# theislab/dca

Measured on NVIDIA H100. Metric: cells/sec (ZINB AE epoch, device-timed), higher is better.
Workload: dtype bf16-gemm/f32-acc/f32-loss

## Files before the change

dca_b200/_lib.py:

```python
from __future__ import annotations

import ctypes as C
import os

_HERE = os.path.dirname(os.path.abspath(__file__))
LIB_PATH = os.path.join(_HERE, "libdca_b200.so")

DCA_MAX_HIDDEN = 8
DCA_NAME_LEN = 48

ACTIVATION_IDS = {"relu": 0, "linear": 1, "elu": 2, "selu": 3, "tanh": 4, "sigmoid": 5, "hard_sigmoid": 6,
                  "softplus": 7, "softsign": 8, "exponential": 9, "LeakyReLU": 10, "PReLU": 11}
OPTIMIZERS = {"RMSprop": (0, 1e-3), "SGD": (1, 1e-2), "Adagrad": (2, 1e-2), "Adadelta": (3, 1.0), "Adam": (4, 1e-3),
              "Adamax": (5, 2e-3), "Nadam": (6, 2e-3)}
OPTIMIZERS.update({k.lower(): v for k, v in list(OPTIMIZERS.items())})
AE_TYPE_IDS = {"zinb-conddisp": 0, "zinb": 1, "nb-conddisp": 2, "nb": 3,
               "poisson": 4, "normal": 5, "nb-shared": 6, "zinb-shared": 7, "zinb-elempi": 8, "nb-fork": 9, "zinb-fork": 10}
F32, BF16 = 0, 1
GEMM_AUTO, GEMM_GENERIC, GEMM_TCGEN05 = 0, 1, 2
REGION_PARAMS, REGION_GRADS, REGION_RMS, REGION_BN_STATE, REGION_EPOCH_ACC = 0, 1, 2, 3, 4


class DcaError(RuntimeError):
    pass
# ... 61 lines not shown
    "dca_train_step_host": (C.c_int, [_vp, _vp, _vp, _vp, _i32, _f, _f, C.POINTER(_f), _vp]),
    "dca_set_input_transform": (C.c_int, [_vp, _vp, _vp, _i32, _i32, _vp]),
    "dca_set_loss_ring": (C.c_int, [_vp, _vp, _i32]),
    "dca_stream_begin": (C.c_int, [_vp, _vp, _i64, _vp, _i64, _i32, _vp]),
    "dca_stream_begin_packed": (C.c_int, [_vp, _vp, _i32, _i64, _vp, _vp, _vp, _i64, _i32, _vp]),
    "dca_stream_begin_sparse": (C.c_int, [_vp, _vp, _vp, _vp, _vp, _vp, _vp, _i64, _i32, _vp]),
    "dca_stream_step": (C.c_int, [_vp, _i64, _i64, _vp]),
    "dca_stream_end": (C.c_int, [_vp, _vp]),
    "dca_expand_packed_counts": (C.c_int, [_vp, _i32, _vp, _vp, _vp, _i32, _i32, _vp, _vp, _i32, _i32, _vp, _vp, _i32, _vp,
                                           _vp]),
    "dca_expand_sparse_counts": (C.c_int, [_vp, _vp, _vp, _i32, _vp, _vp, _vp, _i32, _i32, _vp, _vp, _i32, _i32, _vp, _vp,
                                           _i32, _vp, _vp]),
    "dca_zinb_loss_fwd_bwd": (C.c_int, [_vp, _i64, _vp, _vp, _vp, _vp, _vp, _i64, _i32, _i32, _i32, _f, _f,
                                        _vp, _vp, _vp, _i32, _vp, _vp, _vp, _sz, _vp]),
    "dca_zinb_loss_workspace_bytes": (C.c_int, [_i32, _i32, C.POINTER(_sz)]),
    "dca_zinb_loss_fwd": (C.c_int, [_vp, _i64, _vp, _vp, _vp, _vp, _vp, _i64, _i32, _i32, _i32, _f,
                                    _vp, _vp, _sz, _vp]),
    "dca_zinb_elem_host": (C.c_int, [_i32, _f, _f, _f, _f, _f, _f, C.POINTER(_f * 4)]),
    "dca_dropout_mask_host": (C.c_int, [C.c_uint64, C.c_uint64, _i32, _i64, _f, _vp]),
    "dca_activation_host": (C.c_int, [_i32, _f, _f, C.POINTER(_f * 2)]),
    "dca_activation_bwd_host": (C.c_int, [_i32, _f, _f, _f, _i32, _f, C.POINTER(_f * 2)]),
    "dca_dense_heads_fwd": (C.c_int, [_vp, _i64, _i32, _i32, _i32, _vp, _vp, _vp, _vp, _vp, _vp, _vp,
                                      _vp, _vp, _vp, _i64, _vp]),
    "dca_tc_heads_fwd": (C.c_int, [_vp, _i32, _vp, _vp, _i32, _i32, C.POINTER(_i32 * 3), _vp, _vp, _vp, _vp, _i64, _vp]),
    "dca_tc_heads_loss": (C.c_int, [_vp, _i32, _vp, _vp, _i32, _vp, _i64, _vp, _vp, _f, _f, _vp, _vp, _vp, _i64, _vp,
                                    _vp, _sz, _vp]),
    "dca_tc_gene_gemm": (C.c_int, [_i32, _vp, _vp, _vp, _i64, _i32, _i32, _i32, _vp, _vp, _vp, _vp, _vp, _vp, _i64, _i32,
                                   _vp, _vp, _vp, _vp]),
    "dca_tc_gene_gemm_sms": (C.c_int, [_i32, _vp, _vp, _vp, _i64, _i32, _i32, _i32, _vp, _vp, _vp, _vp, _vp, _vp, _i64,
                                       _i32, _vp, _vp, _vp, _vp, _i32]),
    "dca_tc_gene_gemm_rows": (C.c_int, [_i32, _vp, _vp, _vp, _i64, _vp, _i32, _i32, _i32, _vp, _vp, _vp, _vp, _vp, _vp,
                                        _i64, _i32, _vp, _vp, _vp, _vp, _i32]),
    "dca_head_bwd_schedule": (C.c_int, [_i32, _i32, _i32, _i32, _i32, _vp, _i64, C.POINTER(_i64), _vp]),
    "dca_enc_bwd_schedule": (C.c_int, [_i32, _i32, _vp, _i64, _vp]),
    "dca_tc_probe": (C.c_int, [_vp, _i32, _i32, _vp, _i32, _i32, _i32, _i32, _i32, _i32, _i32, _i32, _i32, _i32, _i32,
                               _vp, _vp]),
    "dca_profile_enable": (C.c_int, [_vp, _i32]),
    "dca_profile_read": (C.c_int, [_vp, C.POINTER(C.c_double * 6), C.POINTER(C.c_int64 * 6), _i32]),
    "dca_engine_info": (C.c_int, [_vp, C.POINTER(_i32 * 8)]),
    "dca_write_text_matrix": (C.c_int, [C.c_char_p, _vp, _i32, _i64, _i64, _i64, _vp, _vp, _i32, _i32]),
    "dca_write_text_device": (C.c_int, [C.c_char_p, _i32, _vp, _i64, _i64, _i64, _i32, _vp, _i64, _vp, _vp, _i64, _i32, _vp,
                                        _vp]),
    "dca_format_fixed6_host": (C.c_int, [_vp, _i64, _vp, _vp]),
    "dca_read_text_counts": (C.c_int, [C.c_char_p, _i32, _i32, _i64, _i32, _vp, _vp, _i64, _vp, _vp, _i64, _vp]),
    "dca_read_mtx_counts": (C.c_int, [C.c_char_p, _i32, _i64, _i32, _vp, _vp, _vp, _vp, _vp]),
    "dca_read_text_counts_gz": (C.c_int, [C.c_char_p, _i32, _i32, _i64, _i32, _vp, _vp, _i64, _vp, _vp, _i64, _vp]),
    "dca_read_mtx_counts_gz": (C.c_int, [C.c_char_p, _i32, _i64, _i32, _vp, _vp, _vp, _vp, _vp]),
    "dca_gunzip": (C.c_int, [C.c_char_p, _i32, _vp, _vp, _i64, _vp]),
    "dca_inflate_span_host": (C.c_int, [_vp, _i64, _i32, _i64, _i64, _vp, _i64, _vp]),
    "dca_inflate_find_host": (C.c_int, [_vp, _i64, _i64, _i64, _vp]),
    "dca_count_escapes": (C.c_int, [_vp, _i32, _i64, _i64, _i64, _vp, _i32]),
    "dca_pack_counts": (C.c_int, [_vp, _i32, _i64, _i64, _i64, _i32, _vp, _vp, _vp, _i32]),
    "dca_sparse_counts": (C.c_int, [_vp, _i32, _i64, _i64, _i64, _vp, _vp, _i32]),
    "dca_pack_sparse": (C.c_int, [_vp, _i32, _i64, _i64, _i64, _vp, _vp, _vp, _vp, _vp, _i32]),
    "dca_preprocess_workspace_bytes": (C.c_int, [_i64, _i32, C.POINTER(_sz)]),
    "dca_counts_csr_to_dense": (C.c_int, [_vp, _vp, _vp, _i64, _i32, _vp, _i64, _vp]),
    "dca_count_totals": (C.c_int, [_vp, _i64, _i64, _i32, _vp, _vp, _vp, _vp, _sz, _vp]),
    "dca_gather_counts": (C.c_int, [_vp, _i64, _vp, _i64, _vp, _i32, _vp, _i64, _vp]),
    "dca_log_moments": (C.c_int, [_vp, _i64, _i64, _i32, _vp, C.c_double, _i32, _vp, _vp, _vp, _sz, _vp]),
    "dca_normalize_write": (C.c_int, [_vp, _i64, _i64, _i32, _vp, C.c_double, _i32, _vp, _vp, _vp, _i32, _i64, _vp]),
    "dca_stats_workspace_bytes": (C.c_int, [_i64, _i32, _i64, C.POINTER(_sz)]),
    "dca_stats_begin": (C.c_int, [_i64, _i32, _vp, _sz, _vp]),
    "dca_count_totals_rows": (C.c_int, [_vp, _i64, _i64, _i64, _i64, _i32, _vp, _vp, _sz, _vp]),
    "dca_count_totals_finish": (C.c_int, [_i64, _i32, _vp, _vp, _vp, _sz, _vp]),
    "dca_log_moments_rows": (C.c_int, [_i32, _vp, _i64, _i64, _i64, _i64, _i32, _vp, C.c_double, _i32, _vp, _vp, _sz,
                                       _vp]),
# ... 58 lines not shown
```

dca_b200/csrc/gene_gemm_tc.cu:

```cuda
#include "engine.h"
#include "tc_common.cuh"

namespace dca {
namespace tc {
int g_gg_profile = 0;
int g_head_bwd_banded = 1;
int g_head_bwd_stagger = 1300;
namespace gg {

constexpr int kThreads = 256;
constexpr uint32_t kZBytes = 128 * 128 * 2;
constexpr uint32_t kWBytes = 64 * 128 * 2;
constexpr uint32_t kHBytes = 128 * 64 * 2;
constexpr uint32_t kOutBytes = 128 * 64 * 4;
constexpr uint32_t kOnesBytes = 16 * 128;
constexpr int kMaxGb = 4;
constexpr int kMaxSlots = 16;

static_assert(kWBytes == kHBytes, "the two item kinds of the banded launch share one stage shape");
template <bool DO_A, bool DO_B, bool BANDED>
constexpr int stages() { return DO_A && DO_B && !BANDED ? 2 : 3; }
template <bool DO_A, bool DO_B, bool BANDED>
constexpr uint32_t stage_bytes() { return BANDED ? kZBytes + kWBytes : kZBytes + (DO_B ? kWBytes : 0) + (DO_A ? kHBytes : 0); }
template <bool DO_A, bool DO_B, bool COLSUM, bool BANDED>
constexpr uint32_t smem_bytes() {
  return stages<DO_A, DO_B, BANDED>() * stage_bytes<DO_A, DO_B, BANDED>() + (DO_A ? kOutBytes : 0) + (COLSUM ? kOnesBytes : 0) + 1024;
}

struct BandItem { int kind, head, gr, gb0, ng, cb0, ncb; };

__host__ __device__ inline BandItem band_item(int k, int n_gb, int n_cb, int gpr, int ranges) {
  const int per_head = n_gb + ranges * n_cb, full_band = gpr + n_cb;
  BandItem it;
  it.head = k / per_head; k -= it.head * per_head;
  it.gr = min(k / full_band, ranges - 1); k -= it.gr * full_band;
  const int gb0 = it.gr * gpr, ng = min(n_gb, gb0 + gpr) - gb0, m = min(ng, n_cb);
  int idx;
  if (k < 2 * m) { it.kind = k & 1; idx = k >> 1; }
  else { it.kind = ng > n_cb ? 0 : 1; idx = k - m; }
  if (it.kind == 0) { it.gb0 = gb0 + idx; it.ng = 1; it.cb0 = 0; it.ncb = n_cb; }
  else { it.gb0 = gb0; it.ng = ng; it.cb0 = idx; it.ncb = 1; }
  return it;
}

struct Params {
  int B, G, n_heads;
  int n_cb, n_gb;
  int gb_per_item, cb_per_item;
  int gene_ranges, cell_splits;
  int total_items;
  int stagger;
  float* db[3];
  float* part; int64_t part_stride;
  const int32_t* rows; const __nv_bfloat16* zsrc; int64_t ldz;
};

__device__ __forceinline__ void cp_async_16(uint32_t smem_dst, const void* src, uint32_t src_bytes) {
  asm volatile("cp.async.cg.shared.global [%0], [%1], 16, %2;" ::"r"(smem_dst), "l"(src), "r"(src_bytes) : "memory");
}
__device__ __forceinline__ void cp_async_commit() { asm volatile("cp.async.commit_group;" ::: "memory"); }
template <int N>
__device__ __forceinline__ void cp_async_wait() { asm volatile("cp.async.wait_group %0;" ::"n"(N) : "memory"); }

template <bool DO_A, bool DO_B, bool COLSUM, bool WK, int MAXG, bool BANDED>
__global__ void __launch_bounds__(kThreads, 1)
gene_gemm_kernel(const __grid_constant__ CUtensorMap map_z0, const __grid_constant__ CUtensorMap map_z1,
                 const __grid_constant__ CUtensorMap map_z2, const __grid_constant__ CUtensorMap map_h,
                 const __grid_constant__ CUtensorMap map_w0, const __grid_constant__ CUtensorMap map_w1,
                 const __grid_constant__ CUtensorMap map_w2, const __grid_constant__ CUtensorMap map_dw0, const __grid_constant__ CUtensorMap map_dw1,
                 const __grid_constant__ CUtensorMap map_dw2, const int dw_transposed, const Params p) {
  static_assert(!BANDED || (DO_A && DO_B && MAXG == 1), "banded items hold one gene block of (a) accumulators");
  constexpr int kStages = stages<DO_A, DO_B, BANDED>();
  constexpr uint32_t kStage = stage_bytes<DO_A, DO_B, BANDED>();
  constexpr uint32_t kHOff = kZBytes + (DO_B && !BANDED ? kWBytes : 0);
  extern __shared__ __align__(1024) uint8_t smem_raw[];
  uint8_t* smem = smem_raw + ((1024u - (smem_u32(smem_raw) & 1023u)) & 1023u);
  uint8_t* s_st = smem;
  float* s_o = reinterpret_cast<float*>(s_st + kStages * kStage);
  uint8_t* s_ones = reinterpret_cast<uint8_t*>(s_o) + (DO_A ? kOutBytes : 0);
  __shared__ uint64_t full[kStages];

  if (threadIdx.x == 0) {
    for (int i = 0; i < kStages; ++i) mbar_init(&full[i], 1);
    fence_barrier_init();
// ... 220 lines not shown
    const float4 v = __ldcs(reinterpret_cast<const float4*>(part + sl * stride + i));
    acc.x += v.x; acc.y += v.y; acc.z += v.z; acc.w += v.w;
  }
  *reinterpret_cast<float4*>(out + i) = acc;
}

void plan_a(Params& p, int n_heads, int sm_count) {
  int best_gpi = 1; long long best_cost = -1;
  for (int gpi = 1; gpi <= kMaxGb; ++gpi) {
    const long long items = (long long)cdiv(p.n_gb, gpi) * n_heads, rounds = (items + sm_count - 1) / sm_count;
    const long long cost = rounds * ((long long)gpi * p.n_cb + 2ll * gpi);
    if (best_cost < 0 || cost < best_cost) { best_cost = cost; best_gpi = gpi; }
  }
  p.gb_per_item = best_gpi; p.gene_ranges = cdiv(p.n_gb, best_gpi);
  p.cb_per_item = p.n_cb; p.cell_splits = 1;
  p.total_items = p.gene_ranges * n_heads;
}
void plan_b(Params& p, int n_heads, int sm_count) {
  p.cb_per_item = 1; p.cell_splits = p.n_cb;
  int gsplits = cdiv(4 * sm_count, p.n_cb * n_heads); if (gsplits < 1) gsplits = 1;
  if (gsplits > kMaxSlots / n_heads) gsplits = kMaxSlots / n_heads;
  if (gsplits > p.n_gb) gsplits = p.n_gb;
  while (gsplits > 1 && cdiv(p.n_gb, gsplits) < 4) --gsplits;
  p.gb_per_item = cdiv(p.n_gb, gsplits); p.gene_ranges = cdiv(p.n_gb, p.gb_per_item);
  p.total_items = p.gene_ranges * p.cell_splits * n_heads;
}
void plan_banded(Params& p, int n_heads, int sm_count, int* grid) {
  plan_b(p, n_heads, sm_count);
  p.total_items = n_heads * (p.n_gb + p.gene_ranges * p.n_cb);
  const int band = p.gb_per_item + p.n_cb;
  *grid = min(p.total_items, sm_count >= band ? sm_count / band * band : sm_count);
}

constexpr int kEbMaxW = 3;
constexpr int kEbThreads = 128 * kEbMaxW;
constexpr uint32_t kEbSub = 128 * 128;
constexpr uint32_t kEbStage = kEbMaxW * kEbSub + kHBytes;
constexpr int kEbStages = 3;
constexpr uint32_t kEbSmem = kEbStages * kEbStage + 1024;
static_assert(kEbMaxW * 64 * 64 * 4 <= kEbStage, "the flush staging tiles fit in the first stage");

struct EncBwdParams {
  int B, G, n_cb, n_blk;
  const int32_t* rows; const __nv_bfloat16* zsrc; int64_t ldz;
};

__host__ __device__ inline int eb_first(int c, int n_blk, int ctas) { return c * (n_blk / ctas) + min(c, n_blk % ctas); }
inline int eb_ctas(int n_blk, int sm_count) { return max(1, min(sm_count, n_blk)); }

__global__ void __launch_bounds__(kEbThreads, 1)
gene_gemm_enc_bwd_kernel(const __grid_constant__ CUtensorMap map_z, const __grid_constant__ CUtensorMap map_h,
                         const __grid_constant__ CUtensorMap map_dw, const int dw_transposed, const EncBwdParams p) {
  extern __shared__ __align__(1024) uint8_t smem_raw[];
  uint8_t* s_st = smem_raw + ((1024u - (smem_u32(smem_raw) & 1023u)) & 1023u);
  __shared__ uint64_t full[kEbStages];
  if (threadIdx.x == 0) {
    for (int i = 0; i < kEbStages; ++i) mbar_init(&full[i], 1);
    fence_barrier_init();
  }
  __syncthreads();

  const int wg = threadIdx.x >> 7, w = (threadIdx.x >> 5) & 3, l = threadIdx.x & 31;
  const int frow = 16 * w + (l >> 2), fcol = 2 * (l & 3);
  const bool gather = p.rows != nullptr;
  const int g_r0 = (threadIdx.x & 127) >> 3, g_c = threadIdx.x & 7;
  const uint32_t g_dst = wg * kEbSub + g_r0 * 128 + ((g_c ^ (g_r0 & 7)) << 4);
  int src_row[8];

  const int last = eb_first(blockIdx.x + 1, p.n_blk, gridDim.x);
  uint32_t T0 = 0;
  for (int blk0 = eb_first(blockIdx.x, p.n_blk, gridDim.x); blk0 < last; blk0 += kEbMaxW) {
    const int nw = min(kEbMaxW, last - blk0);
    const bool mine = wg < nw;
    if (threadIdx.x == 0) bulk_wait_read<0>();
    __syncthreads();

    auto issue = [&](int t) {
      const int st = (T0 + t) % kEbStages;
      uint8_t* dst = s_st + st * kEbStage;
      mbar_expect_tx(&full[st], kHBytes + (gather ? 0u : nw * kEbSub));
// ... 111 lines not shown
    for (int i = 0; i < 3; ++i) {
      float* d = dW[i < n_heads ? i : 0];
      if (dW_transposed) DCA_TRY(make_tensor_map_2d(&mdw[i], d, 4, 0, 64, (uint64_t)G, (uint64_t)dW_ld, 64, 128, 0));
      else {
        if (dW_ld != 64) { set_error("gene_gemm_tc: non-transposed dW needs ld == 64"); return DCA_ERR_BAD_ARG; }
        DCA_TRY(make_tensor_map_2d(&mdw[i], d, 4, 0, (uint64_t)G, 64, 64, 128, 64, 0));
      }
    }
  }
  if (do_b) {
    for (int i = 0; i < 3; ++i) {
      const __nv_bfloat16* w = W[i < n_heads ? i : 0];
      if (mode == 3) DCA_TRY(make_tensor_map_2d(&mw[i], w, 2, 1, 64, (uint64_t)G, (uint64_t)G, 64, 64, 1));
      else DCA_TRY(make_tensor_map_2d(&mw[i], w, 2, 1, (uint64_t)G, 64, 64, 128, 64, 1));
    }
  }
  Params base{};
  base.B = B; base.G = G; base.n_heads = n_heads;
  base.n_cb = cdiv(B, 128); base.n_gb = cdiv(G, 128);
  for (int i = 0; i < 3; ++i) base.db[i] = db ? db[i] : nullptr;
  base.part = reinterpret_cast<float*>(ws); base.part_stride = (int64_t)base.n_cb * 128 * 64;
  base.rows = rows; base.zsrc = Z[0]; base.ldz = ldz;

#define DCA_GG_LAUNCH(P, GRID, A, Bb, Cc, WKk, MG, BND)                                                                \
  do {                                                                                                                 \
    static bool attr = false;                                                                                          \
    constexpr uint32_t sm = smem_bytes<A, Bb, Cc, BND>();                                                              \
    if (!attr) { DCA_CUDA_OK(cudaFuncSetAttribute(gene_gemm_kernel<A, Bb, Cc, WKk, MG, BND>, cudaFuncAttributeMaxDynamicSharedMemorySize, (int)sm)); attr = true; } \
    gene_gemm_kernel<A, Bb, Cc, WKk, MG, BND><<<GRID, kThreads, sm, s>>>(mz[0], mz[1], mz[2], mh, mw[0], mw[1], mw[2],  \
                                                                          mdw[0], mdw[1], mdw[2], dW_transposed, P);  \
    DCA_LAUNCH_CHECK();                                                                                                \
  } while (0)

  if (mode == 3 && g_head_bwd_banded) {
    Params p = base;
    int grid = 0;
    plan_banded(p, n_heads, sm_count, &grid);
    p.stagger = g_head_bwd_stagger;
    DCA_GG_LAUNCH(p, grid, true, true, true, true, 1, true);
    const int64_t n = (int64_t)B * 64;
    gene_gemm_reduce_kernel<<<(unsigned)cdiv(n / 4, 256), 256, 0, s>>>(p.part, p.gene_ranges * n_heads, p.part_stride, out_b, n);
    DCA_LAUNCH_CHECK();
    return DCA_OK;
  }
  if (mode == 2) {
    EncBwdParams p{B, G, base.n_cb, cdiv(G, 64), rows, Z[0], ldz};
    CUtensorMap mdw64;
    if (dW_transposed) DCA_TRY(make_tensor_map_2d(&mdw64, dW[0], 4, 0, 64, (uint64_t)G, (uint64_t)dW_ld, 64, 64, 0));
    else DCA_TRY(make_tensor_map_2d(&mdw64, dW[0], 4, 0, (uint64_t)G, 64, 64, 64, 64, 0));
    static bool attr = false;
    if (!attr) { DCA_CUDA_OK(cudaFuncSetAttribute(gene_gemm_enc_bwd_kernel, cudaFuncAttributeMaxDynamicSharedMemorySize, (int)kEbSmem)); attr = true; }
    gene_gemm_enc_bwd_kernel<<<eb_ctas(p.n_blk, sm_count), kEbThreads, kEbSmem, s>>>(mz[0], mh, mdw64, dW_transposed, p);
    DCA_LAUNCH_CHECK();
    return DCA_OK;
  }
  if (do_a) {
    Params p = base;
    plan_a(p, n_heads, sm_count);
    DCA_GG_LAUNCH(p, min(p.total_items, sm_count), true, false, true, false, kMaxGb, false);
  }
  if (do_b) {
    Params p = base;
    plan_b(p, n_heads, sm_count);
    const int grid = min(p.total_items, sm_count);
    if (mode == 3) DCA_GG_LAUNCH(p, grid, false, true, false, true, 1, false);
    else DCA_GG_LAUNCH(p, grid, false, true, false, false, 1, false);
    const int64_t n = (int64_t)B * 64;
    gene_gemm_reduce_kernel<<<(unsigned)cdiv(n / 4, 256), 256, 0, s>>>(p.part, p.gene_ranges * n_heads, p.part_stride, out_b, n);
    DCA_LAUNCH_CHECK();
  }
#undef DCA_GG_LAUNCH
  return DCA_OK;
}

}
}

using namespace dca;
extern "C" int dca_tc_gene_gemm_rows(int32_t mode, const void* Z0, const void* Z1, const void* Z2, int64_t ldz,
                                     const int32_t* rows, int32_t batch, int32_t genes, int32_t n_heads, const void* H,
                                     const void* W, float* out_b, float* dW0, float* dW1, float* dW2, int64_t dW_ld,
                                     int32_t dW_transposed, float* db0, float* db1, float* db2, void* stream, int32_t sm_count) {
  if (!Z0 || batch <= 0 || genes <= 0 || n_heads < 1 || n_heads > 3) { set_error("dca_tc_gene_gemm: bad argument"); return DCA_ERR_BAD_ARG; }
  int dev = 0, sms = 132;
  cudaGetDevice(&dev);
  cudaDeviceGetAttribute(&sms, cudaDevAttrMultiProcessorCount, dev);
  if (sm_count > 0 && sm_count < sms) sms = sm_count;
  const __nv_bfloat16* Z[3] = {(const __nv_bfloat16*)Z0, (const __nv_bfloat16*)Z1, (const __nv_bfloat16*)Z2};
// ... 42 lines not shown
  if (banded) {
    tc::gg::Params p = base;
    plan_banded(p, n_heads, sm_count, &grid[0]);
    grid[1] = 0;
    for (int i = 0; i < p.total_items; ++i) {
      const tc::gg::BandItem it = tc::gg::band_item(i, p.n_gb, p.n_cb, p.gb_per_item, p.gene_ranges);
      put(0, it.kind, it.head, it.gb0, it.ng, it.cb0, it.ncb, it.kind ? it.head * p.gene_ranges + it.gr : -1);
    }
  } else {
    tc::gg::Params pa = base, pb = base;
    plan_a(pa, n_heads, sm_count);
    plan_b(pb, n_heads, sm_count);
    grid[0] = std::min(pa.total_items, (int)sm_count); grid[1] = std::min(pb.total_items, (int)sm_count);
    for (int pass = 0; pass < 2; ++pass) {
      const tc::gg::Params& p = pass ? pb : pa;
      for (int i = 0; i < p.total_items; ++i) {
        const int cs = i % p.cell_splits, r = i / p.cell_splits, gr = r % p.gene_ranges, head = r / p.gene_ranges;
        const int gb0 = gr * p.gb_per_item, cb0 = cs * p.cb_per_item;
        put(pass, pass, head, gb0, std::min(p.n_gb, gb0 + p.gb_per_item) - gb0, cb0, std::min(p.n_cb, cb0 + p.cb_per_item) - cb0,
            pass ? head * p.gene_ranges + gr : -1);
      }
    }
  }
  *n_items = k;
  return DCA_OK;
}
extern "C" int dca_enc_bwd_schedule(int32_t genes, int32_t sm_count, int32_t* first, int64_t cap, int32_t* ctas) {
  if (genes <= 0 || sm_count < 1 || !ctas) { set_error("dca_enc_bwd_schedule: bad argument"); return DCA_ERR_BAD_ARG; }
  const int n_blk = cdiv(genes, 64);
  *ctas = tc::gg::eb_ctas(n_blk, sm_count);
  for (int64_t c = 0; first && c < cap && c <= *ctas; ++c) first[c] = tc::gg::eb_first((int)c, n_blk, *ctas);
  return DCA_OK;
}
```

dca_b200/csrc/zinb_loss.cu:

```cuda
#include "dca_internal.cuh"
#include <string>
#include "zinb_math.cuh"
#include "tc_common.cuh"
#include "head_act.cuh"
#include <cstdlib>

namespace dca {
namespace tc { extern int g_gg_profile; extern int g_head_bwd_banded; extern int g_head_bwd_stagger; }

namespace {

constexpr int kThreads = 256;
constexpr int kVec = 4;
constexpr int kColsPerBlock = kThreads * kVec;
constexpr int kMaxBlocks = 65536;

struct LossTune { int target_blocks; unsigned producer_sleep_ns, consumer_sleep_ns; int branch_free; int ring; };
LossTune g_tune = {0 , 0u, 0u, 1 ,
                   1 };

int sm_count_cached() {
  static int n = 0;
  if (!n) { int dev = 0; if (cudaGetDevice(&dev) != cudaSuccess || cudaDeviceGetAttribute(&n, cudaDevAttrMultiProcessorCount, dev) != cudaSuccess || n <= 0) n = 132; }
  return n;
}

struct Plan { int col_blocks, rows_per_block, row_chunks; };

inline Plan make_plan(int B, int G, int cols_per_block, int max_rpb = 1 << 30) {
  Plan p;
  p.col_blocks = cdiv(G, cols_per_block);
  const int target = g_tune.target_blocks > 0 ? g_tune.target_blocks
                     : ((long long)B * G <= (32ll << 20) ? 3 * sm_count_cached() : 16 * sm_count_cached());
  int chunks = target / p.col_blocks;
  if (chunks < 1) chunks = 1;
  if (chunks > B) chunks = B;
  int rpb = cdiv(B, chunks);
  if (rpb < 2 && B >= 2) rpb = 2;
  if (rpb > max_rpb) rpb = max_rpb;
  while ((long long)cdiv(B, rpb) * p.col_blocks > kMaxBlocks && rpb < max_rpb) ++rpb;
  p.rows_per_block = rpb;
// ... 1082 lines not shown
  p.nblk = cdiv(B, 64);
  const long long units = (long long)cdiv(G, 128) * p.nblk;
  if (units > INT_MAX) { set_error("heads_loss_tc: %lld (gene tile, cell block) units, over 2^31 - 1", units); return DCA_ERR_BAD_ARG; }
  p.units = (int)units;
  p.ridge = a.ridge; p.inv_n = a.inv_n;
  p.loss_partial = reinterpret_cast<double*>(a.ws); p.lf = lf_dev;
  FoldArgs fa{reinterpret_cast<unsigned*>(reinterpret_cast<char*>(a.ws) + sizeof(double) * (size_t)kMaxBlocks), a.loss_sum,
              a.fin_penalty, a.fin_loss_slot, a.fin_epoch_acc, a.fin_batch};
  if (!a.counter_ready) DCA_CUDA_OK(cudaMemsetAsync(fa.counter, 0, sizeof(unsigned), s));
  static bool attr = false;
  if (!attr) { DCA_CUDA_OK(cudaFuncSetAttribute(heads_loss_kernel, cudaFuncAttributeMaxDynamicSharedMemorySize, (int)kSmemBytes)); attr = true; }
  const int grid = (int)std::min<long long>(p.units, sm_count_cached());
  heads_loss_kernel<<<grid, kCtaThreads, kSmemBytes, s>>>(mh, mw[0], mw[1], mw[2], p, fa);
  DCA_LAUNCH_CHECK();
  return DCA_OK;
}

}

using namespace dca;

extern "C" int dca_set_tunable(const char* name, int64_t value) {
  if (!name) { set_error("dca_set_tunable: null name"); return DCA_ERR_BAD_ARG; }
  const std::string n(name);
  if (n == "loss_target_blocks" && value >= 0 && value <= kMaxBlocks) g_tune.target_blocks = (int)value;
  else if (n == "loss_producer_sleep_ns" && value >= 0 && value <= 100000) g_tune.producer_sleep_ns = (unsigned)value;
  else if (n == "loss_consumer_sleep_ns" && value >= 0 && value <= 100000) g_tune.consumer_sleep_ns = (unsigned)value;
  else if (n == "fused_heads" && (value == 0 || value == 1)) g_fused_heads_default = (int)value;
  else if (n == "loss_branch_free" && (value == 0 || value == 1)) g_tune.branch_free = (int)value;
  else if (n == "loss_ring" && value >= 0 && value <= 2) g_tune.ring = (int)value;
  else if (n == "gg_profile" && (value == 0 || value == 1)) tc::g_gg_profile = (int)value;
  else if (n == "head_bwd_banded" && (value == 0 || value == 1)) tc::g_head_bwd_banded = (int)value;
  else if (n == "head_bwd_stagger" && value >= 0 && value <= 100000) tc::g_head_bwd_stagger = (int)value;
  else { set_error("dca_set_tunable: unknown name or value out of range (%s = %lld)", name, (long long)value); return DCA_ERR_BAD_ARG; }
  return DCA_OK;
}

extern "C" int dca_zinb_loss_workspace_bytes(int32_t batch, int32_t genes, size_t* bytes) {
  if (!bytes || batch <= 0 || genes <= 0) { set_error("dca_zinb_loss_workspace_bytes: bad argument"); return DCA_ERR_BAD_ARG; }
  *bytes = loss_workspace_bytes(batch, genes);
  return DCA_OK;
}

extern "C" int dca_zinb_loss_fwd_bwd(const float* Y, int64_t ldy, const int32_t* rows, const float* sf,
                                     const float* m, const float* d, const float* pi, int64_t ld,
                                     int32_t batch, int32_t genes, int32_t ae_type, float ridge, float inv_n,
                                     void* dzm, void* dzd, void* dzp, int32_t grad_dtype, float* dtheta,
                                     double* loss_sum, void* workspace, size_t workspace_bytes, void* stream) {
  if (ae_type < 0 || ae_type > 3) { set_error("dca_zinb_loss_fwd_bwd: unknown ae_type %d", ae_type); return DCA_ERR_BAD_ARG; }
  LossArgs a{Y, ldy, rows, sf, m, d, pi, ld, batch, genes, ae_type, ridge, inv_n, dzm, dzd, dzp,
             grad_dtype == DCA_BF16 ? 1 : 0, dtheta, loss_sum, workspace, workspace_bytes};
  return zinb_loss_fwd_bwd(a, (cudaStream_t)stream);
}

extern "C" int dca_tc_heads_loss(const void* Hb, int32_t batch, const void* Wk, const float* bias, int32_t genes,
                                 const float* Y, int64_t ldy, const int32_t* rows, const float* sf, float ridge, float inv_n,
                                 void* dzm, void* dzd, void* dzp, int64_t ldz, double* loss_sum, void* workspace,
                                 size_t workspace_bytes, void* stream) {
  if (!Hb || !Wk || !bias || !Y || !dzm || !dzd || !dzp || !loss_sum || batch <= 0 || genes <= 0) {
    set_error("dca_tc_heads_loss: bad argument"); return DCA_ERR_BAD_ARG;
  }
  HeadsLossArgs a{};
  a.H3 = (const __nv_bfloat16*)Hb; a.B = batch; a.G = genes;
  for (int i = 0; i < 3; ++i) { a.W[i] = (const __nv_bfloat16*)Wk + (size_t)i * 64 * genes; a.bias[i] = bias + (size_t)i * genes; }
  a.Y = Y; a.ldy = ldy; a.rows = rows; a.sf = sf; a.ridge = ridge; a.inv_n = inv_n;
  a.dz[0] = (__nv_bfloat16*)dzm; a.dz[1] = (__nv_bfloat16*)dzd; a.dz[2] = (__nv_bfloat16*)dzp; a.ldz = ldz;
// ... 65 lines not shown
```

include/dca_b200.h:

```cpp
#ifndef DCA_B200_H
#define DCA_B200_H

#include <stddef.h>
#include <stdint.h>

#ifdef __cplusplus
extern "C" {
#endif

#define DCA_B200_VERSION 100
#define DCA_MAX_HIDDEN 8
#define DCA_NAME_LEN 48

typedef enum dca_status {
  DCA_OK = 0,
  DCA_ERR_BAD_ARG = -1,
  DCA_ERR_CUDA = -2,
  DCA_ERR_UNSUPPORTED = -3,
  DCA_ERR_NONFINITE = -4,
  DCA_ERR_NO_DEVICE = -5
} dca_status;

typedef enum dca_ae_type {
  DCA_AE_ZINB_CONDDISP = 0,
// ... 210 lines not shown
int dca_activation_host(int32_t act, float x, float alpha, float out[2]);
int dca_activation_bwd_host(int32_t act, float x, float alpha, float rate, int32_t kept, float g, float out[2]);

int dca_dense_heads_fwd(const float* H, int64_t ldh, int32_t batch, int32_t K, int32_t genes,
                        const float* w_mean, const float* b_mean,
                        const float* w_disp, const float* b_disp,
                        const float* w_pi, const float* b_pi,
                        const float* row_scale,
                        float* m_out, float* d_out, float* pi_out, int64_t ld_out, void* stream);

int dca_tc_heads_fwd(const void* Hb, int32_t batch, const void* Wk, const float* bias, int32_t genes,
                     int32_t n_heads, const int32_t kind[3], const float* row_scale,
                     float* out0, float* out1, float* out2, int64_t ld_out, void* stream);

int dca_tc_heads_loss(const void* Hb, int32_t batch, const void* Wk, const float* bias, int32_t genes,
                      const float* Y, int64_t ldy, const int32_t* rows, const float* sf, float ridge, float inv_n,
                      void* dzm, void* dzd, void* dzp, int64_t ldz, double* loss_sum, void* workspace,
                      size_t workspace_bytes, void* stream);

int dca_tc_gene_gemm(int32_t mode, const void* Z0, const void* Z1, const void* Z2, int64_t ldz, int32_t batch,
                     int32_t genes, int32_t n_heads, const void* H, const void* W, float* out_b,
                     float* dW0, float* dW1, float* dW2, int64_t dW_ld, int32_t dW_transposed,
                     float* db0, float* db1, float* db2, void* stream);
int dca_tc_gene_gemm_sms(int32_t mode, const void* Z0, const void* Z1, const void* Z2, int64_t ldz, int32_t batch,
                         int32_t genes, int32_t n_heads, const void* H, const void* W, float* out_b,
                         float* dW0, float* dW1, float* dW2, int64_t dW_ld, int32_t dW_transposed,
                         float* db0, float* db1, float* db2, void* stream, int32_t sm_count);
int dca_tc_gene_gemm_rows(int32_t mode, const void* Z0, const void* Z1, const void* Z2, int64_t ldz, const int32_t* rows,
                          int32_t batch, int32_t genes, int32_t n_heads, const void* H, const void* W, float* out_b,
                          float* dW0, float* dW1, float* dW2, int64_t dW_ld, int32_t dW_transposed,
                          float* db0, float* db1, float* db2, void* stream, int32_t sm_count);
int dca_head_bwd_schedule(int32_t batch, int32_t genes, int32_t n_heads, int32_t sm_count, int32_t banded,
                          int32_t* items, int64_t cap, int64_t* n_items, int32_t* grid);
int dca_enc_bwd_schedule(int32_t genes, int32_t sm_count, int32_t* first, int64_t cap, int32_t* ctas);

#define DCA_PRE_SIZE_FACTORS 1
#define DCA_PRE_LOG1P 2
#define DCA_PRE_SCALE 4
int dca_preprocess_workspace_bytes(int64_t n_cells, int32_t genes, size_t* bytes);
int dca_counts_csr_to_dense(const int64_t* indptr, const int32_t* indices, const float* data, int64_t n_cells,
                            int32_t genes, float* Y, int64_t ldy, void* stream);
int dca_count_totals(const float* Y, int64_t ldy, int64_t n_cells, int32_t genes, double* cell_totals,
                     double* gene_totals, int64_t* n_bad, void* workspace, size_t workspace_bytes, void* stream);
int dca_gather_counts(const float* Y, int64_t ldy, const int32_t* rows, int64_t n_rows, const int32_t* cols,
                      int32_t n_cols, float* out, int64_t ldo, void* stream);
int dca_log_moments(const float* Y, int64_t ldy, int64_t n_cells, int32_t genes, const double* n_counts, double median,
                    int32_t flags, double* mean, double* std, void* workspace, size_t workspace_bytes, void* stream);
int dca_normalize_write(const float* Y, int64_t ldy, int64_t n_cells, int32_t genes, const double* n_counts,
                        double median, int32_t flags, const double* mean, const double* std, void* X, int32_t x_dtype,
                        int64_t ldx, void* stream);
int dca_stats_workspace_bytes(int64_t n_cells, int32_t genes, int64_t max_chunk_rows, size_t* bytes);
int dca_stats_begin(int64_t n_cells, int32_t genes, void* workspace, size_t workspace_bytes, void* stream);
int dca_count_totals_rows(const float* Y, int64_t ldy, int64_t row0, int64_t n_rows, int64_t n_cells, int32_t genes,
                          double* cell_totals, void* workspace, size_t workspace_bytes, void* stream);
int dca_count_totals_finish(int64_t n_cells, int32_t genes, double* gene_totals, int64_t* n_bad, void* workspace,
                            size_t workspace_bytes, void* stream);
int dca_log_moments_rows(int32_t pass, const float* Y, int64_t ldy, int64_t row0, int64_t n_rows, int64_t n_cells,
                         int32_t genes, const double* n_counts, double median, int32_t flags, const double* mean,
                         void* workspace, size_t workspace_bytes, void* stream);
int dca_log_moments_finish(int32_t pass, int64_t n_cells, int32_t genes, int32_t flags, double* out, void* workspace,
                           size_t workspace_bytes, void* stream);

int dca_tc_probe(const void* A, int32_t a_rows, int32_t a_cols, const void* B, int32_t b_rows, int32_t b_cols,
                 int32_t a_mn_major, int32_t b_mn_major, int32_t M, int32_t N, int32_t K,
                 int32_t a_lbo, int32_t a_sbo, int32_t b_lbo, int32_t b_sbo, float* D, void* stream);

// ... 52 lines not shown
```

Baseline: 3.198 million.

## Add thread-block-cluster head backward kernel chaining dH partials via DSMEM

Adds a new head-backward GEMM kernel launched as thread-block clusters. Each CTA keeps a few gene blocks of W resident and accumulates dW and db locally, and passes the partial dH accumulator to the next CTA in the cluster through distributed shared memory with remote mbarriers. Only the last CTA in each chain writes the partial to global memory. This is meant to remove the separate banded work items and cut global partial traffic, in exchange for serialising across cluster ranks, keeping W resident in shared memory and depending on cluster occupancy. It is on by default and falls back to the banded path when the cluster fit test fails.

New measurement: 3.231 million (median of 6 runs). 1.01x the previous value.

```diff
diff --git a/dca_b200/_lib.py b/dca_b200/_lib.py
--- a/dca_b200/_lib.py
+++ b/dca_b200/_lib.py
@@ -117,6 +117,8 @@
     "dca_tc_gene_gemm_rows": (C.c_int, [_i32, _vp, _vp, _vp, _i64, _vp, _i32, _i32, _i32, _vp, _vp, _vp, _vp, _vp, _vp,
                                         _i64, _i32, _vp, _vp, _vp, _vp, _i32]),
     "dca_head_bwd_schedule": (C.c_int, [_i32, _i32, _i32, _i32, _i32, _vp, _i64, C.POINTER(_i64), _vp]),
+    "dca_head_bwd_cluster_schedule": (C.c_int, [_i32, _i32, _i32, _i32, _i32, _vp, _i64, C.POINTER(_i64), C.POINTER(_i32)]),
+    "dca_head_bwd_last_path": (_i32, []),
     "dca_enc_bwd_schedule": (C.c_int, [_i32, _i32, _vp, _i64, _vp]),
     "dca_tc_probe": (C.c_int, [_vp, _i32, _i32, _vp, _i32, _i32, _i32, _i32, _i32, _i32, _i32, _i32, _i32, _i32, _i32,
                                _vp, _vp]),
diff --git a/dca_b200/csrc/gene_gemm_tc.cu b/dca_b200/csrc/gene_gemm_tc.cu
--- a/dca_b200/csrc/gene_gemm_tc.cu
+++ b/dca_b200/csrc/gene_gemm_tc.cu
@@ -6,6 +6,8 @@
 int g_gg_profile = 0;
 int g_head_bwd_banded = 1;
 int g_head_bwd_stagger = 1300;
+int g_head_bwd_cluster = 1;
+int g_head_bwd_path = -1;
 namespace gg {
 
 constexpr int kThreads = 256;
@@ -50,6 +52,7 @@
   int gene_ranges, cell_splits;
   int total_items;
   int stagger;
+  int cluster;
   float* db[3];
   float* part; int64_t part_stride;
   const int32_t* rows; const __nv_bfloat16* zsrc; int64_t ldz;
@@ -336,6 +339,256 @@
   *grid = min(p.total_items, sm_count >= band ? sm_count / band * band : sm_count);
 }
 
+__host__ __device__ inline int eb_first(int c, int n_blk, int ctas) { return c * (n_blk / ctas) + min(c, n_blk % ctas); }
+
+constexpr int kClMaxCtas = 8;
+constexpr int kClStages = 3;
+constexpr uint32_t kClHOff = kMaxGb * kWBytes;
+constexpr uint32_t kClZOff = kClHOff + 2 * kHBytes;
+constexpr uint32_t kClXOff = kClZOff + kClStages * kZBytes;
+constexpr uint32_t kClOnesOff = kClXOff + kThreads * 32 * 4;
+constexpr uint32_t kClBytes = kClOnesOff + kOnesBytes;
+constexpr int kClBars = kClStages + 2 + 1 + 2;
+constexpr uint32_t kClSmem = kClBytes + 1024;
+static_assert(kClSmem <= 232448, "one CTA per SM: at most 227 KB of shared memory");
+static_assert(kClBars * 8 <= 1024 / 2, "the mbarriers fit before or after the 1024-aligned region");
+
+__device__ __forceinline__ uint32_t cluster_map(uint32_t addr, uint32_t rank) {
+  uint32_t r;
+  asm volatile("mapa.shared::cluster.u32 %0, %1, %2;" : "=r"(r) : "r"(addr), "r"(rank));
+  return r;
+}
+__device__ __forceinline__ void cluster_sync() {
+  asm volatile("barrier.cluster.arrive.release.aligned;\n\tbarrier.cluster.wait.acquire.aligned;" ::: "memory");
+}
+__device__ __forceinline__ void st_cluster_f4(uint32_t addr, float a, float b, float c, float d) {
+  asm volatile("st.shared::cluster.v4.f32 [%0], {%1, %2, %3, %4};" ::"r"(addr), "f"(a), "f"(b), "f"(c), "f"(d) : "memory");
+}
+__device__ __forceinline__ void mbar_arrive_remote(uint32_t cluster_addr) {
+  asm volatile("mbarrier.arrive.release.cluster.shared::cluster.b64 _, [%0];" ::"r"(cluster_addr) : "memory");
+}
+__device__ __forceinline__ void mbar_wait_cluster(uint64_t* bar, uint32_t parity) {
+  uint32_t polls = 0, ok;
+  long long t0 = 0;
+  for (;;) {
+    asm volatile(
+        "{\n\t.reg .pred p;\n\t"
+        "mbarrier.try_wait.parity.acquire.cluster.shared::cta.b64 p, [%1], %2;\n\t"
+        "selp.u32 %0, 1, 0, p;\n\t}"
+        : "=r"(ok) : "r"(smem_u32(bar)), "r"(parity) : "memory");
+    if (ok) return;
+    if ((++polls & 0x3FFF) == 0) {
+      const long long now = clock64();
+      if (t0 == 0) t0 = now;
+      else if (now - t0 > 4000000000ll) __trap();
+    }
+  }
+}
+
+__global__ void __launch_bounds__(kThreads, 1)
+gene_gemm_cluster_kernel(const __grid_constant__ CUtensorMap map_z0, const __grid_constant__ CUtensorMap map_z1,
+                         const __grid_constant__ CUtensorMap map_z2, const __grid_constant__ CUtensorMap map_h,
+                         const __grid_constant__ CUtensorMap map_w0, const __grid_constant__ CUtensorMap map_w1,
+                         const __grid_constant__ CUtensorMap map_w2, const __grid_constant__ CUtensorMap map_dw0,
+                         const __grid_constant__ CUtensorMap map_dw1, const __grid_constant__ CUtensorMap map_dw2,
+                         const int dw_transposed, const Params p) {
+  extern __shared__ __align__(1024) uint8_t smem_raw[];
+  const uint32_t pad = (1024u - (smem_u32(smem_raw) & 1023u)) & 1023u;
+  uint8_t* smem = smem_raw + pad;
+  uint64_t* bars = reinterpret_cast<uint64_t*>(pad >= kClBars * 8 ? smem_raw : smem + kClBytes);
+  uint64_t* zfull = bars;
+  uint64_t* hfull = zfull + kClStages;
+  uint64_t* wfull = hfull + 2;
+  uint64_t* xfull = wfull + 1;
+  uint64_t* xfree = xfull + 1;
+  const float4* s_x = reinterpret_cast<const float4*>(smem + kClXOff);
+  const uint32_t s_ones = smem_u32(smem + kClOnesOff);
+  const int tid = threadIdx.x;
+
+  const int q = blockIdx.x % p.cluster, band = blockIdx.x / p.cluster;
+  const int head = band / p.gene_ranges, gr = band % p.gene_ranges;
+  const int gb0 = gr * p.gb_per_item, ng = min(p.n_gb, gb0 + p.gb_per_item) - gb0, nq = min(ng, p.cluster);
+  const int own0 = q < nq ? gb0 + eb_first(q, ng, nq) : 0, nown = q < nq ? eb_first(q + 1, ng, nq) - eb_first(q, ng, nq) : 0;
+  const bool first = q == 0, last = q == nq - 1;
+
+  if (tid == 0) {
+    for (int i = 0; i < kClStages; ++i) mbar_init(&zfull[i], 1);
+    mbar_init(&hfull[0], 1); mbar_init(&hfull[1], 1); mbar_init(wfull, 1);
+    mbar_init(xfull, kThreads); mbar_init(xfree, 1);
+    fence_barrier_init();
+  }
+  for (int i = tid; i < (int)kOnesBytes / 4; i += kThreads) reinterpret_cast<uint32_t*>(smem + kClOnesOff)[i] = 0x3F803F80u;
+  fence_proxy_async_smem();
+  cluster_sync();
+
+  if (nown > 0) {
+    const int wg = tid >> 7, w = (tid >> 5) & 3, l = tid & 31;
+    const int frow = 16 * w + (l >> 2), fcol = 2 * (l & 3);
+    const CUtensorMap* mz = head == 0 ? &map_z0 : (head == 1 ? &map_z1 : &map_z2);
+    const CUtensorMap* mw = head == 0 ? &map_w0 : (head == 1 ? &map_w1 : &map_w2);
+    const CUtensorMap* mdw = head == 0 ? &map_dw0 : (head == 1 ? &map_dw1 : &map_dw2);
+    const int n_tiles = p.n_cb * nown;
+
+    auto issue_z = [&](int t) {
+      const int st = t % kClStages, gb = own0 + t % nown, cb = t / nown;
+      uint8_t* dst = smem + kClZOff + st * kZBytes;
+      mbar_expect_tx(&zfull[st], kZBytes);
+      tma_load_2d(dst, mz, gb * 128, cb * 128, &zfull[st]);
+      tma_load_2d(dst + kZBytes / 2, mz, gb * 128 + 64, cb * 128, &zfull[st]);
+    };
+    auto issue_h = [&](int cb) {
+      mbar_expect_tx(&hfull[cb & 1], kHBytes);
+      tma_load_2d(smem + kClHOff + (cb & 1) * kHBytes, &map_h, 0, cb * 128, &hfull[cb & 1]);
+    };
+    if (tid == 0) {
+      mbar_expect_tx(wfull, nown * kWBytes);
+      for (int i = 0; i < nown; ++i) {
+        tma_load_2d(smem + i * kWBytes, mw, (own0 + i) * 128, 0, wfull);
+        tma_load_2d(smem + i * kWBytes + kWBytes / 2, mw, (own0 + i) * 128 + 64, 0, wfull);
+      }
+      issue_h(0);
+      for (int t = 0; t < kClStages - 1 && t < n_tiles; ++t) issue_z(t);
+    }
+
+    float acc_a[kMaxGb][32], acc_c[kMaxGb][8], acc_b[32];
+#pragma unroll
+    for (int j = 0; j < kMaxGb; ++j) {
+#pragma unroll
+      for (int i = 0; i < 32; ++i) acc_a[j][i] = 0.f;
+#pragma unroll
+      for (int i = 0; i < 8; ++i) acc_c[j][i] = 0.f;
+    }
+    mbar_wait(wfull, 0);
+
+    int t = 0;
+    for (int cb = 0; cb < p.n_cb; ++cb) {
+      if (tid == 0 && cb + 1 < p.n_cb) issue_h(cb + 1);
+      mbar_wait(&hfull[cb & 1], (cb >> 1) & 1);
+      const uint32_t hb = smem_u32(smem + kClHOff + (cb & 1) * kHBytes);
+#pragma unroll
+      for (int i = 0; i < kMaxGb; ++i) {
+        if (i >= nown) break;
+        if (tid == 0 && t + kClStages - 1 < n_tiles) issue_z(t + kClStages - 1);
+        const int st = t % kClStages;
+        mbar_wait(&zfull[st], (t / kClStages) & 1);
+        const uint32_t zb = smem_u32(smem + kClZOff + st * kZBytes), wb = smem_u32(smem + i * kWBytes);
+        wgmma_fence();
+#pragma unroll
+        for (int k = 0; k < 8; ++k) {
+          const uint64_t da = make_smem_desc(zb + wg * (kZBytes / 2) + k * 2048, 0, 1024);
+          wgmma_m64n64k16<1, 1>(acc_a[i], da, make_smem_desc(hb + k * 2048, 0, 1024), 1u);
+          wgmma_m64n16k16<1, 0>(acc_c[i], da, make_smem_desc(s_ones + (k & 3) * 32, 0, 1024), 1u);
+        }
+        if (i == 0) {
+          if (first) {
+#pragma unroll
+            for (int r = 0; r < 32; ++r) acc_b[r] = 0.f;
+          } else {
+            mbar_wait_cluster(xfull, cb & 1);
+#pragma unroll
+            for (int r = 0; r < 8; ++r) {
+              const float4 v = s_x[r * kThreads + tid];
+              acc_b[4 * r] = v.x; acc_b[4 * r + 1] = v.y; acc_b[4 * r + 2] = v.z; acc_b[4 * r + 3] = v.w;
+            }
+          }
+          wgmma_fence();
+        }
+#pragma unroll
+        for (int h = 0; h < 2; ++h)
+#pragma unroll
+          for (int k = 0; k < 4; ++k)
+            wgmma_m64n64k16<0, 0>(acc_b, make_smem_desc(zb + h * (kZBytes / 2) + wg * 64 * 128 + k * 32, 0, 1024),
+                                  make_smem_desc(wb + h * (kWBytes / 2) + k * 32, 0, 1024), 1u);
+        wgmma_commit();
+        wgmma_wait<0>();
+        acc_fence(acc_b);
+#pragma unroll
+        for (int jj = 0; jj < kMaxGb; ++jj) { acc_fence(acc_a[jj]); acc_fence(acc_c[jj]); }
+        __syncthreads();
+        if (i == 0 && !first && tid == 0) mbar_arrive_remote(cluster_map(smem_u32(xfree), q - 1));
+        ++t;
+      }
+      if (last) {
+        float* dst = p.part + (int64_t)(head * p.gene_ranges + gr) * p.part_stride + (int64_t)cb * 128 * 64;
+#pragma unroll
+        for (int i = 0; i < 32; i += 2) {
+          const int row = wg * 64 + frow + 8 * ((i >> 1) & 1), col = 8 * (i >> 2) + fcol;
+          *reinterpret_cast<float2*>(dst + row * 64 + col) = make_float2(acc_b[i], acc_b[i + 1]);
+        }
+      } else {
+        if (cb > 0) mbar_wait_cluster(xfree, (cb - 1) & 1);
+        const uint32_t dst = cluster_map(smem_u32(smem + kClXOff), q + 1) + tid * 16;
+#pragma unroll
+        for (int r = 0; r < 8; ++r)
+          st_cluster_f4(dst + r * kThreads * 16, acc_b[4 * r], acc_b[4 * r + 1], acc_b[4 * r + 2], acc_b[4 * r + 3]);
+        mbar_arrive_remote(cluster_map(smem_u32(xfull), q + 1));
+      }
+    }
+
+    float* s_o = reinterpret_cast<float*>(smem + kClZOff);
+#pragma unroll
+    for (int j = 0; j < kMaxGb; ++j) {
+      if (j >= nown) break;
+      const int gb = own0 + j;
+      if (tid == 0) bulk_wait_read<0>();
+      __syncthreads();
+      if (dw_transposed) {
+#pragma unroll
+        for (int i = 0; i < 32; ++i) {
+          const int g = wg * 64 + frow + 8 * ((i >> 1) & 1), f = 8 * (i >> 2) + fcol + (i & 1);
+          s_o[f * 128 + g] = acc_a[j][i];
+        }
+      } else {
+#pragma unroll
+        for (int i = 0; i < 32; i += 2) {
+          const int g = wg * 64 + frow + 8 * ((i >> 1) & 1), f = 8 * (i >> 2) + fcol;
+          *reinterpret_cast<float2*>(s_o + g * 64 + f) = make_float2(acc_a[j][i], acc_a[j][i + 1]);
+        }
+      }
+      fence_proxy_async_smem();
+      __syncthreads();
+      if (tid == 0) {
+        tma_reduce_add_2d(mdw, dw_transposed ? gb * 128 : 0, dw_transposed ? 0 : gb * 128, s_o);
+        bulk_commit();
+      }
+      float* dbh = head == 0 ? p.db[0] : (head == 1 ? p.db[1] : p.db[2]);
+      if ((l & 3) == 0 && dbh) {
+        const int g = gb * 128 + wg * 64 + frow;
+        if (g < p.G) atomicAdd(dbh + g, acc_c[j][0]);
+        if (g + 8 < p.G) atomicAdd(dbh + g + 8, acc_c[j][2]);
+      }
+    }
+    if (tid == 0) bulk_wait<0>();
+  }
+  cluster_sync();
+}
+
+inline int cluster_ctas(const Params& p, int n_heads, int sm_count, int max_clusters) {
+  const int c = cdiv(p.gb_per_item, kMaxGb), bands = n_heads * p.gene_ranges;
+  return c <= kClMaxCtas && bands * c <= sm_count && bands <= max_clusters ? c : 0;
+}
+int cluster_occupancy(int ctas) {
+  static int cache[kClMaxCtas + 1] = {};
+  static bool attr = false;
+  if (ctas < 1 || ctas > kClMaxCtas) return 0;
+  if (cache[ctas] == 0) {
+    if (!attr) {
+      if (cudaFuncSetAttribute(gene_gemm_cluster_kernel, cudaFuncAttributeMaxDynamicSharedMemorySize, (int)kClSmem) != cudaSuccess) return 0;
+      attr = true;
+    }
+    cudaLaunchConfig_t cfg = {};
+    cudaLaunchAttribute at[1];
+    at[0].id = cudaLaunchAttributeClusterDimension;
+    at[0].val.clusterDim.x = ctas; at[0].val.clusterDim.y = 1; at[0].val.clusterDim.z = 1;
+    cfg.gridDim = dim3(ctas); cfg.blockDim = dim3(kThreads); cfg.dynamicSmemBytes = kClSmem;
+    cfg.attrs = at; cfg.numAttrs = 1;
+    int n = 0;
+    if (cudaOccupancyMaxActiveClusters(&n, gene_gemm_cluster_kernel, &cfg) != cudaSuccess) { cudaGetLastError(); return 0; }
+    cache[ctas] = n > 0 ? n : -1;
+  }
+  return cache[ctas] > 0 ? cache[ctas] : 0;
+}
+
 constexpr int kEbMaxW = 3;
 constexpr int kEbThreads = 128 * kEbMaxW;
 constexpr uint32_t kEbSub = 128 * 128;
@@ -349,7 +602,6 @@
   const int32_t* rows; const __nv_bfloat16* zsrc; int64_t ldz;
 };
 
-__host__ __device__ inline int eb_first(int c, int n_blk, int ctas) { return c * (n_blk / ctas) + min(c, n_blk % ctas); }
 inline int eb_ctas(int n_blk, int sm_count) { return max(1, min(sm_count, n_blk)); }
 
 __global__ void __launch_bounds__(kEbThreads, 1)
@@ -527,6 +779,28 @@
     DCA_LAUNCH_CHECK();                                                                                                \
   } while (0)
 
+  if (mode == 3 && g_head_bwd_banded && g_head_bwd_cluster) {
+    Params p = base;
+    plan_b(p, n_heads, sm_count);
+    const int c = cluster_ctas(p, n_heads, sm_count, cluster_occupancy(cdiv(p.gb_per_item, kMaxGb)));
+    if (c > 0) {
+      p.cluster = c; p.total_items = n_heads * p.gene_ranges;
+      cudaLaunchConfig_t cfg = {};
+      cudaLaunchAttribute at[1];
+      at[0].id = cudaLaunchAttributeClusterDimension;
+      at[0].val.clusterDim.x = c; at[0].val.clusterDim.y = 1; at[0].val.clusterDim.z = 1;
+      cfg.gridDim = dim3(p.total_items * c); cfg.blockDim = dim3(kThreads); cfg.dynamicSmemBytes = kClSmem; cfg.stream = s;
+      cfg.attrs = at; cfg.numAttrs = 1;
+      DCA_CUDA_OK(cudaLaunchKernelEx(&cfg, gene_gemm_cluster_kernel, mz[0], mz[1], mz[2], mh, mw[0], mw[1], mw[2], mdw[0],
+                                     mdw[1], mdw[2], (int)dW_transposed, p));
+      DCA_LAUNCH_CHECK();
+      const int64_t n = (int64_t)B * 64;
+      gene_gemm_reduce_kernel<<<(unsigned)cdiv(n / 4, 256), 256, 0, s>>>(p.part, p.gene_ranges * n_heads, p.part_stride, out_b, n);
+      DCA_LAUNCH_CHECK();
+      g_head_bwd_path = 2;
+      return DCA_OK;
+    }
+  }
   if (mode == 3 && g_head_bwd_banded) {
     Params p = base;
     int grid = 0;
@@ -536,6 +810,7 @@
     const int64_t n = (int64_t)B * 64;
     gene_gemm_reduce_kernel<<<(unsigned)cdiv(n / 4, 256), 256, 0, s>>>(p.part, p.gene_ranges * n_heads, p.part_stride, out_b, n);
     DCA_LAUNCH_CHECK();
+    g_head_bwd_path = 1;
     return DCA_OK;
   }
   if (mode == 2) {
@@ -549,6 +824,7 @@
     DCA_LAUNCH_CHECK();
     return DCA_OK;
   }
+  if (mode == 3) g_head_bwd_path = 0;
   if (do_a) {
     Params p = base;
     plan_a(p, n_heads, sm_count);
@@ -657,3 +933,27 @@
   for (int64_t c = 0; first && c < cap && c <= *ctas; ++c) first[c] = tc::gg::eb_first((int)c, n_blk, *ctas);
   return DCA_OK;
 }
+extern "C" int dca_head_bwd_cluster_schedule(int32_t batch, int32_t genes, int32_t n_heads, int32_t sm_count,
+                                             int32_t max_clusters, int32_t* ctas, int64_t cap, int64_t* n_ctas,
+                                             int32_t* cluster) {
+  if (batch <= 0 || genes <= 0 || n_heads < 1 || n_heads > 3 || sm_count < 1 || !n_ctas || !cluster) {
+    set_error("dca_head_bwd_cluster_schedule: bad argument"); return DCA_ERR_BAD_ARG;
+  }
+  tc::gg::Params p{};
+  p.n_cb = cdiv(batch, 128); p.n_gb = cdiv(genes, 128);
+  tc::gg::plan_b(p, n_heads, sm_count);
+  const int want = cdiv(p.gb_per_item, tc::gg::kMaxGb);
+  const int c = tc::gg::cluster_ctas(p, n_heads, sm_count, max_clusters >= 0 ? max_clusters : tc::gg::cluster_occupancy(want));
+  *cluster = c;
+  *n_ctas = (int64_t)n_heads * p.gene_ranges * c;
+  for (int64_t k = 0; ctas && k < cap && k < *n_ctas; ++k) {
+    const int q = (int)(k % c), band = (int)(k / c), head = band / p.gene_ranges, gr = band % p.gene_ranges;
+    const int gb0 = gr * p.gb_per_item, ng = std::min(p.n_gb, gb0 + p.gb_per_item) - gb0, nq = std::min(ng, c);
+    const int f = q < nq ? tc::gg::eb_first(q, ng, nq) : 0, n = q < nq ? tc::gg::eb_first(q + 1, ng, nq) - f : 0;
+    int32_t* r = ctas + 8 * k;
+    r[0] = band; r[1] = head; r[2] = gr; r[3] = head * p.gene_ranges + gr; r[4] = q;
+    r[5] = n ? gb0 + f : -1; r[6] = n; r[7] = q == nq - 1;
+  }
+  return DCA_OK;
+}
+extern "C" int32_t dca_head_bwd_last_path(void) { return tc::g_head_bwd_path; }
diff --git a/dca_b200/csrc/zinb_loss.cu b/dca_b200/csrc/zinb_loss.cu
--- a/dca_b200/csrc/zinb_loss.cu
+++ b/dca_b200/csrc/zinb_loss.cu
@@ -6,7 +6,7 @@
 #include <cstdlib>
 
 namespace dca {
-namespace tc { extern int g_gg_profile; extern int g_head_bwd_banded; extern int g_head_bwd_stagger; }
+namespace tc { extern int g_gg_profile; extern int g_head_bwd_banded; extern int g_head_bwd_stagger; extern int g_head_bwd_cluster; }
 
 namespace {
 
@@ -1155,6 +1155,7 @@
   else if (n == "gg_profile" && (value == 0 || value == 1)) tc::g_gg_profile = (int)value;
   else if (n == "head_bwd_banded" && (value == 0 || value == 1)) tc::g_head_bwd_banded = (int)value;
   else if (n == "head_bwd_stagger" && value >= 0 && value <= 100000) tc::g_head_bwd_stagger = (int)value;
+  else if (n == "head_bwd_cluster" && (value == 0 || value == 1)) tc::g_head_bwd_cluster = (int)value;
   else { set_error("dca_set_tunable: unknown name or value out of range (%s = %lld)", name, (long long)value); return DCA_ERR_BAD_ARG; }
   return DCA_OK;
 }
diff --git a/include/dca_b200.h b/include/dca_b200.h
--- a/include/dca_b200.h
+++ b/include/dca_b200.h
@@ -266,6 +266,9 @@
                           float* db0, float* db1, float* db2, void* stream, int32_t sm_count);
 int dca_head_bwd_schedule(int32_t batch, int32_t genes, int32_t n_heads, int32_t sm_count, int32_t banded,
                           int32_t* items, int64_t cap, int64_t* n_items, int32_t* grid);
+int dca_head_bwd_cluster_schedule(int32_t batch, int32_t genes, int32_t n_heads, int32_t sm_count, int32_t max_clusters,
+                                  int32_t* ctas, int64_t cap, int64_t* n_ctas, int32_t* cluster);
+int32_t dca_head_bwd_last_path(void);
 int dca_enc_bwd_schedule(int32_t genes, int32_t sm_count, int32_t* first, int64_t cap, int32_t* ctas);
 
 #define DCA_PRE_SIZE_FACTORS 1
```
